# VachaLab/gorder

Measured on AMD Instinct MI355X. Metric: trajectory frames/sec, higher is better.
Workload: dtype f32

## Files before the change

gorder_amd/csrc/kernels_bonds.h:

```cpp
#pragma once

namespace {

__device__ __forceinline__ int grid_index(float x, float lo, float bin, uint32_t n, bool core) {
    const float k = __builtin_roundf(core ? gm_div_core(x - lo, bin) : (x - lo) / bin);
    if (!(k >= 0.0f) || !(k < (float)n)) return -1;
    return (int)k;
}
__device__ __forceinline__ int grid_index_fast(float x, float lo, float inv_bin, uint32_t n) {
    const float k = __builtin_floorf(__builtin_fmaf(x - lo, inv_bin, 0.5f));
    if (!(k >= 0.0f) || !(k < (float)n)) return -1;
    return (int)k;
}
constexpr uint32_t kRecFrames = 4;
struct TiledMapOut {
    uint32_t plane;
    float x0, y0, binx, biny;
    uint32_t nx, ny;
    int bin_core;
    unsigned long long *words;
    unsigned long long *ticks;
};
__device__ __forceinline__ unsigned long long tick_sample_word(int tick, bool lower) {
    return ((unsigned long long)(lower ? 1u : 0u) << 32) | (unsigned long long)(uint32_t)tick;
}
__device__ __forceinline__ unsigned long long map_sample_word(const TiledMapOut &mo, float px, float py, float pz, int tick, bool lower) {
    float x, y;
    if (mo.plane == 0) { x = px; y = py; }
    else if (mo.plane == 1) { x = px; y = pz; }
    else { x = pz; y = py; }
    const int ix = grid_index(x, mo.x0, mo.binx, mo.nx, mo.bin_core != 0), iy = grid_index(y, mo.y0, mo.biny, mo.ny, mo.bin_core != 0);
    if (ix < 0 || iy < 0) return kMapNoSample;
    const uint32_t nt = mo.nx * mo.ny, t = (uint32_t)ix * mo.ny + (uint32_t)iy;
    return ((unsigned long long)((lower ? nt : 0u) + t) << 32) | (unsigned long long)(uint32_t)tick;
}

constexpr uint32_t kNoNan = 0xffffffffu;
struct SampleAcc {
    long long s_tot = 0, s_up = 0;
    uint32_t n_tot = 0, n_up = 0;
};

template <bool ACOS_COS>
__device__ __forceinline__ bool bond_sample(const FrameArgs &a, uint32_t f, float p1x, float p1y, float p1z,
                                            float p2x, float p2y, float p2z, uint32_t mol, SampleAcc &acc,
                                            int &bad, const TiledMapOut *mo = nullptr, unsigned long long *word = nullptr,
                                            unsigned long long *tick_word = nullptr) {
    float vx = p2x - p1x, vy = p2y - p1y, vz = p2z - p1z;
    if (a.pbc) {
        const float *b = a.box9 + 9 * (size_t)f;
        const float bx = b[0], by = b[4], bz = b[8];
        bool slow = false;
        const float rx = gm_min_image_step(vx, bx, slow);
        const float ry = gm_min_image_step(vy, by, slow);
        const float rz = gm_min_image_step(vz, bz, slow);
        if (__builtin_expect(slow, 0)) {
            vx = gm_min_image_loop(vx, bx, bad);
            vy = gm_min_image_loop(vy, by, bad);
            vz = gm_min_image_loop(vz, bz, bad);
        } else {
            vx = rx; vy = ry; vz = rz;
        }
    }
    const float sch = gm_calc_sch<ACOS_COS>(vx, vy, vz, a.nx, a.ny, a.nz, a.n2, a.n2sq);
    const long long tick = gm_tick(sch);
    acc.s_tot += tick;
    acc.n_tot += 1;
    bool lower = false;
    if (a.leaflets) {
        const uint8_t fl = a.aflags[(size_t)a.arow[f] * a.n_mol_total + mol];
        lower = fl != 0;
        if (fl == 0) {
            acc.s_up += tick;
            acc.n_up += 1;
        }
    }
    if (mo) {
        *word = mo->nx == 0u ? tick_sample_word((int)tick, lower)
                             : map_sample_word(*mo, p1x + vx / 2.0f, p1y + vy / 2.0f, p1z + vz / 2.0f, (int)tick, lower);
        if (tick_word) *tick_word = tick_sample_word((int)tick, lower);
    }
    return sch != sch;
}

#ifndef GORDER_COMPUTE_NF
#define GORDER_COMPUTE_NF 8
#endif
typedef float v4f __attribute__((ext_vector_type(4)));

template <int G, int NPF, bool ACOS_COS, bool PBC, bool LEAF, int AXIS = -1>
struct TiledStage {
    static constexpr uint32_t TPF = kBlock / G;

    template <bool TAIL>
    static __device__ __forceinline__ void load(const FrameArgs &a, const Tile &t, uint32_t f0, uint32_t f_end,
                                                uint32_t sk, uint32_t si, v4f (&pre)[NPF]) {
        const uint32_t f = f0 + sk;
        if (TAIL && f >= f_end) return;
        const size_t base = ((size_t)f * a.n_atoms + t.atom0) * 3u;
        const uint32_t n4 = ((uint32_t)(base & 3u) + 3u * t.n_window + 3u) >> 2;
        const v4f *src = reinterpret_cast<const v4f *>(a.xyz + (base & ~(size_t)3));
#pragma unroll
        for (int j = 0; j < NPF; j++) {
            const uint32_t i = si + (uint32_t)j * TPF;
            pre[j] = __builtin_nontemporal_load(src + (i < n4 ? i : n4 - 1u));
        }
    }
    template <bool TAIL, bool FINITE = false>
    static __device__ __forceinline__ bool store(const FrameArgs &a, const Tile &t, uint32_t f0, uint32_t f_end,
                                                 uint32_t sk, uint32_t si, const v4f (&pre)[NPF], float *lds,
                                                 uint32_t lw) {
        const uint32_t f = f0 + sk;
        if (TAIL && f >= f_end) return true;
        const size_t base = ((size_t)f * a.n_atoms + t.atom0) * 3u;
        const uint32_t n4 = ((uint32_t)(base & 3u) + 3u * t.n_window + 3u) >> 2;
        const v4f *src = reinterpret_cast<const v4f *>(a.xyz + (base & ~(size_t)3));
        v4f *dst = reinterpret_cast<v4f *>(lds + (size_t)sk * lw);
        typedef float v2f __attribute__((ext_vector_type(2)));
        v2f poison = {0.0f, 0.0f};
        const v2f zero2 = {0.0f, 0.0f};
#pragma unroll
        for (int j = 0; j < NPF; j++) {
            const uint32_t i = si + (uint32_t)j * TPF;
            if (i < n4) dst[i] = pre[j];
            if (FINITE) {
                poison = __builtin_elementwise_fma(pre[j].xy, zero2, poison);
                poison = __builtin_elementwise_fma(pre[j].zw, zero2, poison);
            }
        }
        for (uint32_t i = si + (uint32_t)NPF * TPF; i < n4; i += TPF) {
            const v4f v = __builtin_nontemporal_load(src + i);
            dst[i] = v;
            if (FINITE) {
                poison = __builtin_elementwise_fma(v.xy, zero2, poison);
                poison = __builtin_elementwise_fma(v.zw, zero2, poison);
            }
        }
        return poison.x + poison.y == 0.0f;
    }
    template <int NF, int OUT = 0>
    static __device__ __forceinline__ void compute_core(const FrameArgs &a, const Tile &t, const Item &it,
                                                        uint32_t f0, const float (&P)[NF][6], SampleAcc &acc,
                                                        int &bad, uint32_t &nan_which, uint32_t &nan_frame,
                                                        const TiledMapOut *mo = nullptr, uint32_t k0 = 0) {
        constexpr bool MAPS = OUT != 0;
        int tick[NF];
        uint8_t fl[NF];
        float bx[NF], by[NF], bz[NF];
        uint32_t rare = 0;
        auto stage_word = [&](int k, float vx, float vy, float vz) {
            mo->words[k0 + (uint32_t)k] = OUT == 2
                ? tick_sample_word(tick[k], LEAF && fl[k] != 0)
                : map_sample_word(*mo, P[k][0] + vx / 2.0f, P[k][1] + vy / 2.0f, P[k][2] + vz / 2.0f, tick[k], LEAF && fl[k] != 0);
            if (OUT == 3) mo->ticks[k0 + (uint32_t)k] = tick_sample_word(tick[k], LEAF && fl[k] != 0);
        };
#pragma unroll
        for (int k = 0; k < NF; k++) {
            if (PBC) {
                const float *b = a.box9 + 9 * (size_t)(f0 + k);
                bx[k] = b[0]; by[k] = b[4]; bz[k] = b[8];
            }
            if (LEAF) fl[k] = a.aflags[(size_t)a.arow[f0 + k] * a.n_mol_total + it.mol];
        }
#pragma unroll
        for (int k = 0; k < NF; k++) {
            float vx = P[k][3] - P[k][0], vy = P[k][4] - P[k][1], vz = P[k][5] - P[k][2];
            bool slow = false;
            if (PBC && AXIS >= 0 && !ACOS_COS && !MAPS) {
                const float ax = __builtin_fabsf(vx), ay = __builtin_fabsf(vy), az = __builtin_fabsf(vz);
                const float tx = bx[k] - ax, ty = by[k] - ay, tz = bz[k] - az;
                vx = ax > bx[k] / 2.0f ? tx : ax;
                vy = ay > by[k] / 2.0f ? ty : ay;
                vz = az > bz[k] / 2.0f ? tz : az;
                slow = __builtin_fminf(__builtin_fminf(tx, ty), tz) < 0.0f;
            } else if (PBC) {
                vx = gm_min_image_step(vx, bx[k], slow);
                vy = gm_min_image_step(vy, by[k], slow);
                vz = gm_min_image_step(vz, bz[k], slow);
            }
            if (AXIS >= 0 && !ACOS_COS) {
                const float sch = gm_sch_axis<AXIS>(vx, vy, vz, slow);
                rare |= (slow ? 1u : 0u) << k;
                tick[k] = gm_tick_finite(sch);
            } else if (AXIS >= 0) {
                const float sch = gm_sch_axis_acos<AXIS>(vx, vy, vz, slow);
                rare |= (slow ? 1u : 0u) << k;
                tick[k] = gm_tick_finite(sch);
            } else {
                bool nonfinite = false;
                const float sch = gm_calc_sch<ACOS_COS, AXIS>(vx, vy, vz, a.nx, a.ny, a.nz, a.n2, a.n2sq, &nonfinite);
                rare |= ((slow || nonfinite || sch != sch) ? 1u : 0u) << k;
                tick[k] = gm_tick(sch);
            }
            if (MAPS) stage_word(k, vx, vy, vz);
        }
        if (__builtin_expect(rare != 0, 0)) {
#pragma unroll
            for (int k = 0; k < NF; k++) {
                if (!((rare >> k) & 1u)) continue;
                float vx = P[k][3] - P[k][0], vy = P[k][4] - P[k][1], vz = P[k][5] - P[k][2];
                if (PBC) {
                    vx = gm_min_image_loop(vx, bx[k], bad);
                    vy = gm_min_image_loop(vy, by[k], bad);
                    vz = gm_min_image_loop(vz, bz[k], bad);
                }
                const float sch = gm_calc_sch<ACOS_COS>(vx, vy, vz, a.nx, a.ny, a.nz, a.n2, a.n2sq);
                tick[k] = gm_tick(sch);
                if (MAPS) stage_word(k, vx, vy, vz);
                if (sch != sch && nan_frame == kNoNan) {
                    if (P[k][0] != P[k][0]) { nan_which = 0; nan_frame = f0 + k; }
                    else if (P[k][3] != P[k][3]) { nan_which = 1; nan_frame = f0 + k; }
                }
            }
        }
        int st = 0, su = 0;
        uint32_t nu = 0;
#pragma unroll
        for (int k = 0; k < NF; k++) {
            st += tick[k];
            if (LEAF) {
                su += fl[k] == 0 ? tick[k] : 0;
                nu += fl[k] == 0 ? 1u : 0u;
            }
        }
        acc.s_tot += st;
        acc.n_tot += NF;
        acc.s_up += su;
        acc.n_up += nu;
    }
    template <int OUT = 0>
    static __device__ __forceinline__ void compute(const FrameArgs &a, const Tile &t, const Item &it, uint32_t f0,
                                                   const float *lds, uint32_t lw, SampleAcc &acc, int &bad,
                                                   uint32_t &nan_which, uint32_t &nan_frame, const TiledMapOut *mo = nullptr) {
        constexpr int NF = (OUT == 1 || OUT == 3 || (OUT == 2 && LEAF)) ? 2 : (GORDER_COMPUTE_NF < G ? GORDER_COMPUTE_NF : G);
#pragma unroll
        for (int h = 0; h < G; h += NF) {
            float P[NF][6];
#pragma unroll
            for (int k = 0; k < NF; k++) {
                const uint32_t sh = (uint32_t)((((size_t)(f0 + h + k) * a.n_atoms + t.atom0) * 3u) & 3u);
                const float *w = lds + (size_t)(h + k) * lw + sh;
                P[k][0] = w[3u * it.li]; P[k][1] = w[3u * it.li + 1]; P[k][2] = w[3u * it.li + 2];
                P[k][3] = w[3u * it.lj]; P[k][4] = w[3u * it.lj + 1]; P[k][5] = w[3u * it.lj + 2];
            }
            compute_core<NF, OUT>(a, t, it, f0 + h, P, acc, bad, nan_which, nan_frame, mo, (uint32_t)h);
        }
    }
    template <int OUT = 0>
    static __device__ __forceinline__ void compute_tail(const FrameArgs &a, const Tile &t, const Item &it,
                                                        uint32_t f0, uint32_t f_end, const float *lds, uint32_t lw,
                                                        SampleAcc &acc, int &bad, uint32_t &nan_which,
                                                        uint32_t &nan_frame, const TiledMapOut *mo = nullptr) {
        if (OUT != 0) {
#pragma unroll
            for (int k = 0; k < G; k++) {
                const uint32_t f = f0 + (uint32_t)k;
                if (f >= f_end) continue;
                const uint32_t sh = (uint32_t)((((size_t)f * a.n_atoms + t.atom0) * 3u) & 3u);
                const float *w = lds + (size_t)k * lw + sh;
                const float p1x = w[3u * it.li], p1y = w[3u * it.li + 1], p1z = w[3u * it.li + 2];
                const float p2x = w[3u * it.lj], p2y = w[3u * it.lj + 1], p2z = w[3u * it.lj + 2];
                if (bond_sample<ACOS_COS>(a, f, p1x, p1y, p1z, p2x, p2y, p2z, it.mol, acc, bad, mo, mo->words + k, OUT == 3 ? mo->ticks + k : nullptr) &&
                    nan_frame == kNoNan) {
                    if (p1x != p1x) { nan_which = 0; nan_frame = f; }
                    else if (p2x != p2x) { nan_which = 1; nan_frame = f; }
                }
            }
            return;
        }
#pragma unroll 1
        for (uint32_t f = f0; f < f_end; f++) {
            const uint32_t sh = (uint32_t)((((size_t)f * a.n_atoms + t.atom0) * 3u) & 3u);
            const float *w = lds + (size_t)(f - f0) * lw + sh;
            const float p1x = w[3u * it.li], p1y = w[3u * it.li + 1], p1z = w[3u * it.li + 2];
            const float p2x = w[3u * it.lj], p2y = w[3u * it.lj + 1], p2z = w[3u * it.lj + 2];
            if (bond_sample<ACOS_COS>(a, f, p1x, p1y, p1z, p2x, p2y, p2z, it.mol, acc, bad) && nan_frame == kNoNan) {
                if (p1x != p1x) { nan_which = 0; nan_frame = f; }
                else if (p2x != p2x) { nan_which = 1; nan_frame = f; }
            }
        }
    }
};

#ifndef GORDER_TILED_MIN_WAVES
#define GORDER_TILED_MIN_WAVES 4
#endif
__device__ __forceinline__ float mom_min(float x, float y) { float r; __asm__("v_min_f32_e32 %0, %1, %2" : "=v"(r) : "v"(x), "v"(y)); return r; }
__device__ __forceinline__ float mom_max(float x, float y) { float r; __asm__("v_max_f32_e32 %0, %1, %2" : "=v"(r) : "v"(x), "v"(y)); return r; }
#define GORDER_MOM_MINMAX_DPP(CTRL_TEXT)                                                                    \
    __asm__("s_nop 1\n\tv_min_f32_dpp %0, %0, %0 " CTRL_TEXT "\n\tv_max_f32_dpp %1, %1, %1 " CTRL_TEXT : "+v"(mn), "+v"(mx))
__device__ __forceinline__ void tiled_moments(const FrameArgs &a, const Tile &t, uint2 own, uint32_t tile_id, uint32_t n_tiles,
                                              uint32_t f, const float *slot, bool finite, uint2 my_head) {
    const uint32_t lane = threadIdx.x & 63u;
    const uint32_t sh = (uint32_t)((((size_t)f * a.n_atoms + t.atom0) * 3u) & 3u);
    const float *w = slot + sh + a.mom_dim + 3u * (own.x - t.atom0);
    const uint32_t n_own = own.y - own.x;
    float s = 0.0f, q = 0.0f, mn = 3.0e38f, mx = -3.0e38f;
    for (uint32_t i0 = 0; i0 < n_own; i0 += 512u) {
        float z[8];
#pragma unroll
        for (uint32_t u = 0; u < 8u; u++) z[u] = w[3u * min(i0 + 64u * u + lane, n_own - 1u)];
#pragma unroll
        for (uint32_t u = 0; u < 8u; u++) {
            if (i0 + 64u * u >= n_own) break;
            float d = z[u];
            if (i0 + 64u * u + 64u > n_own) d = i0 + 64u * u + lane < n_own ? d : 0.0f;
            s += d;
            q = __builtin_fmaf(d, d, q);
            mn = mom_min(mn, z[u]);
            mx = mom_max(mx, z[u]);
        }
    }
#define GORDER_MOM_STEP(CTRL, MASK, CTRL_TEXT)                                                  \
    s += dpp_or_zero<CTRL, MASK>(s); q += dpp_or_zero<CTRL, MASK>(q);                               \
    GORDER_MOM_MINMAX_DPP(CTRL_TEXT);
    GORDER_MOM_STEP(0x111, 0xf, "row_shr:1 row_mask:0xf bank_mask:0xf")
    GORDER_MOM_STEP(0x112, 0xf, "row_shr:2 row_mask:0xf bank_mask:0xf")
    GORDER_MOM_STEP(0x114, 0xf, "row_shr:4 row_mask:0xf bank_mask:0xf")
    GORDER_MOM_STEP(0x118, 0xf, "row_shr:8 row_mask:0xf bank_mask:0xf")
    GORDER_MOM_STEP(0x142, 0xa, "row_bcast:15 row_mask:0xa bank_mask:0xf")
    GORDER_MOM_STEP(0x143, 0xc, "row_bcast:31 row_mask:0xc bank_mask:0xf")
#undef GORDER_MOM_STEP
    const bool all_finite = __all(finite);
    if (lane == 63u) a.mom[(size_t)f * n_tiles + tile_id] = make_float4(all_finite ? s : __builtin_nanf(""), q, mn, mx);
    if (my_head.y != 0xffffffffu) a.head_z[(size_t)f * a.n_mol_total + my_head.y] = slot[sh + a.mom_dim + 3u * my_head.x];
}
template <int G, int NPF, bool ACOS_COS, bool PBC, bool LEAF, int AXIS, bool MOM = false>
__global__ __launch_bounds__(kBlock, GORDER_TILED_MIN_WAVES) void k_bonds_tiled(FrameArgs a_in, const float *__restrict__ xyz,
                                                      const float *__restrict__ box9,
                                                      const uint8_t *__restrict__ aflags,
                                                      const uint32_t *__restrict__ arow,
                                                      const Tile *__restrict__ tiles,
                                                      const Item *__restrict__ items,
                                                      const uint32_t *__restrict__ tile_slots,
                                                      uint32_t n_tiles, uint32_t lw) {
    extern __shared__ __attribute__((aligned(16))) float lds[];
    using S = TiledStage<G, NPF, ACOS_COS, PBC, LEAF, AXIS>;
    FrameArgs a = a_in;
    a.xyz = xyz; a.box9 = box9; a.aflags = aflags; a.arow = arow;
    const uint32_t tile_id = blockIdx.x % n_tiles;
    const uint32_t chunk = blockIdx.x / n_tiles;
    const Tile t = tiles[tile_id];
    const uint32_t tid = threadIdx.x;
    const uint32_t sk = tid / S::TPF, si = tid % S::TPF;
    const bool active = tid < t.n_items;
    Item it{0, 0, 0, 0, 0};
    if (active) it = items[t.item0 + tid];

    const uint32_t f_begin = chunk * a.frames_per_chunk;
    const uint32_t f_end = min(a.n_frames, f_begin + a.frames_per_chunk);
    const uint32_t f_full = f_begin + ((f_end - f_begin) / G) * G;

    SampleAcc acc;
    int bad = 0;
    uint32_t nan_which = 0, nan_frame = kNoNan;
    v4f pre[NPF];
    uint2 own = make_uint2(0u, 0u), my_head = make_uint2(0u, 0xffffffffu);
    if (MOM) {
        own = a.own[tile_id];
        const uint32_t hq = a.own_head_begin[tile_id] + (tid & 63u);
        if (hq < a.own_head_begin[tile_id + 1u]) my_head = a.own_heads[hq];
    }

    if (f_begin < f_full) S::template load<false>(a, t, f_begin, f_end, sk, si, pre);
    for (uint32_t f0 = f_begin; f0 < f_full; f0 += G) {
        const bool finite = S::template store<false, MOM>(a, t, f0, f_end, sk, si, pre, lds, lw);
        __syncthreads();
        if (f0 + G < f_full) S::template load<false>(a, t, f0 + G, f_end, sk, si, pre);
        if (MOM) {
            static_assert(!MOM || (uint32_t)G * 64u == kBlock, "a wave per frame slot");
            tiled_moments(a, t, own, tile_id, n_tiles, f0 + sk, lds + (size_t)sk * lw, finite, my_head);
        }
        if (active) S::compute(a, t, it, f0, lds, lw, acc, bad, nan_which, nan_frame);
        __syncthreads();
    }
    if (f_full < f_end) {
        S::template load<true>(a, t, f_full, f_end, sk, si, pre);
        const bool finite = S::template store<true, MOM>(a, t, f_full, f_end, sk, si, pre, lds, lw);
        __syncthreads();
        if (MOM && f_full + sk < f_end) tiled_moments(a, t, own, tile_id, n_tiles, f_full + sk, lds + (size_t)sk * lw, finite, my_head);
        if (active) S::compute_tail(a, t, it, f_full, f_end, lds, lw, acc, bad, nan_which, nan_frame);
        __syncthreads();
    }

    if (nan_frame != kNoNan)
        raise_error(a.err, GORDER_ERR_UNDEFINED_POSITION, nan_frame, kStageTypes, tile_slots[t.slot0 + it.lslot], 1, it.mol, nan_which);
    if (bad) raise_box_range(a.err, f_begin);

    unsigned long long *l_s = reinterpret_cast<unsigned long long *>(lds);
    uint32_t *l_n = reinterpret_cast<uint32_t *>(l_s + 2 * kBlock);
    l_s[tid] = 0; l_s[kBlock + tid] = 0; l_n[tid] = 0; l_n[kBlock + tid] = 0;
    __syncthreads();
    if (active && acc.n_tot) {
        atomicAdd(&l_s[it.lslot], (unsigned long long)acc.s_tot);
        atomicAdd(&l_n[it.lslot], acc.n_tot);
        if (acc.n_up) {
            atomicAdd(&l_s[kBlock + it.lslot], (unsigned long long)acc.s_up);
            atomicAdd(&l_n[kBlock + it.lslot], acc.n_up);
        }
    }
    __syncthreads();
#ifdef GORDER_DEBUG_NOEPILOGUE
    if (a.n_frames == 0xffffffffu)
#endif
    if (tid < t.n_slots && l_n[tid]) {
        unsigned long long *acc = a.rep + (size_t)(blockIdx.x % a.n_rep) * 4u * a.n_acc;
        const uint32_t slot = tile_slots[t.slot0 + tid];
        atomicAdd(&acc[slot], l_s[tid]);
        atomicAdd(&acc[2u * a.n_acc + slot], (unsigned long long)l_n[tid]);
        if (l_n[kBlock + tid]) {
            atomicAdd(&acc[a.n_acc + slot], l_s[kBlock + tid]);
            atomicAdd(&acc[3u * a.n_acc + slot], (unsigned long long)l_n[kBlock + tid]);
        }
    }
}

template <int G, bool ACOS_COS, bool PBC, bool LEAF>
__global__ __launch_bounds__(kBlock) void k_bonds_gather(FrameArgs a_in, const float *__restrict__ xyz,
                                                       const float *__restrict__ box9,
                                                       const uint8_t *__restrict__ aflags,
                                                       const uint32_t *__restrict__ arow,
                                                       const Tile *__restrict__ tiles,
                                                       const Item *__restrict__ items,
                                                       const uint32_t *__restrict__ tile_slots, uint32_t n_tiles) {
    __shared__ unsigned long long l_s[2 * kBlock];
    __shared__ uint32_t l_n[2 * kBlock];
    using S = TiledStage<G, 1, ACOS_COS, PBC, LEAF>;
    FrameArgs a = a_in;
    a.xyz = xyz; a.box9 = box9; a.aflags = aflags; a.arow = arow;
    const uint32_t tile_id = blockIdx.x % n_tiles;
    const uint32_t chunk = blockIdx.x / n_tiles;
    const Tile t = tiles[tile_id];
    const uint32_t tid = threadIdx.x;
    const bool active = tid < t.n_items;
    Item it{0, 0, 0, 0, 0};
    if (active) it = items[t.item0 + tid];
    const uint32_t f_begin = chunk * a.frames_per_chunk;
    const uint32_t f_end = min(a.n_frames, f_begin + a.frames_per_chunk);
    const uint32_t f_full = f_begin + ((f_end - f_begin) / G) * G;
    const size_t fstride = (size_t)a.n_atoms * 3u;
    const float *pi = xyz + ((size_t)t.atom0 + it.li) * 3u;
    const float *pj = xyz + ((size_t)t.atom0 + it.lj) * 3u;

    SampleAcc acc;
    int bad = 0;
    uint32_t nan_which = 0, nan_frame = kNoNan;
    float cur[G][6], nxt[G][6];
    auto fetch = [&](float (&P)[G][6], uint32_t f0) {
#pragma unroll
        for (int k = 0; k < G; k++) {
            const float *q1 = pi + (size_t)(f0 + k) * fstride, *q2 = pj + (size_t)(f0 + k) * fstride;
            P[k][0] = q1[0]; P[k][1] = q1[1]; P[k][2] = q1[2];
            P[k][3] = q2[0]; P[k][4] = q2[1]; P[k][5] = q2[2];
        }
    };
    if (active) {
        if (f_begin < f_full) fetch(cur, f_begin);
        for (uint32_t f0 = f_begin; f0 < f_full; f0 += G) {
            const bool more = f0 + G < f_full;
            if (more) fetch(nxt, f0 + G);
            S::template compute_core<G>(a, t, it, f0, cur, acc, bad, nan_which, nan_frame);
            if (more) {
#pragma unroll
                for (int k = 0; k < G; k++)
#pragma unroll
                    for (int c = 0; c < 6; c++) cur[k][c] = nxt[k][c];
            }
        }
        for (uint32_t f = f_full; f < f_end; f++) {
            const float *q1 = pi + (size_t)f * fstride, *q2 = pj + (size_t)f * fstride;
            const float p1x = q1[0], p1y = q1[1], p1z = q1[2], p2x = q2[0], p2y = q2[1], p2z = q2[2];
            if (bond_sample<ACOS_COS>(a, f, p1x, p1y, p1z, p2x, p2y, p2z, it.mol, acc, bad) && nan_frame == kNoNan) {
                if (p1x != p1x) { nan_which = 0; nan_frame = f; }
                else if (p2x != p2x) { nan_which = 1; nan_frame = f; }
            }
        }
    }
    if (nan_frame != kNoNan)
        raise_error(a.err, GORDER_ERR_UNDEFINED_POSITION, nan_frame, kStageTypes, tile_slots[t.slot0 + it.lslot], 1, it.mol, nan_which);
    if (bad) raise_box_range(a.err, f_begin);

    l_s[tid] = 0; l_s[kBlock + tid] = 0; l_n[tid] = 0; l_n[kBlock + tid] = 0;
    __syncthreads();
    if (active && acc.n_tot) {
        atomicAdd(&l_s[it.lslot], (unsigned long long)acc.s_tot);
        atomicAdd(&l_n[it.lslot], acc.n_tot);
        if (acc.n_up) {
            atomicAdd(&l_s[kBlock + it.lslot], (unsigned long long)acc.s_up);
            atomicAdd(&l_n[kBlock + it.lslot], acc.n_up);
        }
    }
    __syncthreads();
#ifdef GORDER_DEBUG_NOEPILOGUE
    if (a.n_frames == 0xffffffffu)
#endif
    if (tid < t.n_slots && l_n[tid]) {
        unsigned long long *acc = a.rep + (size_t)(blockIdx.x % a.n_rep) * 4u * a.n_acc;
        const uint32_t slot = tile_slots[t.slot0 + tid];
        atomicAdd(&acc[slot], l_s[tid]);
        atomicAdd(&acc[2u * a.n_acc + slot], (unsigned long long)l_n[tid]);
        if (l_n[kBlock + tid]) {
            atomicAdd(&acc[a.n_acc + slot], l_s[kBlock + tid]);
            atomicAdd(&acc[3u * a.n_acc + slot], (unsigned long long)l_n[kBlock + tid]);
        }
    }
}

template <bool ACOS_COS>
__global__ __launch_bounds__(256) void k_bonds_direct(FrameArgs a, const DirectItem *__restrict__ items,
                                                       uint32_t n_items, uint32_t blocks_per_chunk) {
    const uint32_t chunk = blockIdx.x / blocks_per_chunk;
    const uint32_t q = (blockIdx.x % blocks_per_chunk) * blockDim.x + threadIdx.x;
    if (q >= n_items) return;
    const DirectItem it = items[q];
    const uint32_t f_begin = chunk * a.frames_per_chunk;
    const uint32_t f_end = min(a.n_frames, f_begin + a.frames_per_chunk);
    SampleAcc acc;
    int bad = 0;
    for (uint32_t f = f_begin; f < f_end; f++) {
        const float *p1 = a.xyz + ((size_t)f * a.n_atoms + it.i) * 3u;
        const float *p2 = a.xyz + ((size_t)f * a.n_atoms + it.j) * 3u;
        const float p1x = p1[0], p1y = p1[1], p1z = p1[2];
        const float p2x = p2[0], p2y = p2[1], p2z = p2[2];
        if (__builtin_expect(bond_sample<ACOS_COS>(a, f, p1x, p1y, p1z, p2x, p2y, p2z, it.mol, acc, bad), 0)) {
            if (p1x != p1x) raise_error(a.err, GORDER_ERR_UNDEFINED_POSITION, f, kStageTypes, it.slot, 1, it.mol, 0);
            else if (p2x != p2x) raise_error(a.err, GORDER_ERR_UNDEFINED_POSITION, f, kStageTypes, it.slot, 1, it.mol, 1);
        }
    }
    if (bad) raise_box_range(a.err, f_begin);
    if (acc.n_tot) {
        atomicAdd(&a.acc[it.slot], (unsigned long long)acc.s_tot);
        atomicAdd(&a.acc[2u * a.n_acc + it.slot], (unsigned long long)acc.n_tot);
        if (acc.n_up) {
            atomicAdd(&a.acc[a.n_acc + it.slot], (unsigned long long)acc.s_up);
            atomicAdd(&a.acc[3u * a.n_acc + it.slot], (unsigned long long)acc.n_up);
        }
    }
}

}
```

gorder_amd/csrc/wave_ops.h:

```cpp
#pragma once

namespace {

template <int CTRL, int ROW_MASK = 0xf>
__device__ __forceinline__ int dpp_or_zero(int v) { return __builtin_amdgcn_update_dpp(0, v, CTRL, ROW_MASK, 0xf, true); }
template <int CTRL, int ROW_MASK = 0xf>
__device__ __forceinline__ uint32_t dpp_or_zero(uint32_t v) { return (uint32_t)dpp_or_zero<CTRL, ROW_MASK>((int)v); }
template <int CTRL, int ROW_MASK = 0xf>
__device__ __forceinline__ float dpp_or_zero(float v) { return __int_as_float(dpp_or_zero<CTRL, ROW_MASK>(__float_as_int(v))); }
template <int CTRL, int ROW_MASK = 0xf>
__device__ __forceinline__ double dpp_or_zero(double v) {
    const int lo = dpp_or_zero<CTRL, ROW_MASK>(__double2loint(v)), hi = dpp_or_zero<CTRL, ROW_MASK>(__double2hiint(v));
    return __hiloint2double(hi, lo);
}
template <int CTRL, int ROW_MASK = 0xf>
__device__ __forceinline__ unsigned long long dpp_or_zero(unsigned long long v) {
    const uint32_t lo = dpp_or_zero<CTRL, ROW_MASK>((uint32_t)v), hi = dpp_or_zero<CTRL, ROW_MASK>((uint32_t)(v >> 32));
    return ((unsigned long long)hi << 32) | lo;
}
template <int CTRL, int ROW_MASK = 0xf>
__device__ __forceinline__ float dpp_or_self(float v) {
    return __int_as_float(__builtin_amdgcn_update_dpp(__float_as_int(v), __float_as_int(v), CTRL, ROW_MASK, 0xf, false));
}
__device__ __forceinline__ int lane_value(int v, int l) { return __builtin_amdgcn_readlane(v, l); }
__device__ __forceinline__ uint32_t lane_value(uint32_t v, int l) { return (uint32_t)__builtin_amdgcn_readlane((int)v, l); }
__device__ __forceinline__ float lane_value(float v, int l) { return __int_as_float(__builtin_amdgcn_readlane(__float_as_int(v), l)); }
__device__ __forceinline__ double lane_value(double v, int l) {
    return __hiloint2double(__builtin_amdgcn_readlane(__double2hiint(v), l), __builtin_amdgcn_readlane(__double2loint(v), l));
}
__device__ __forceinline__ unsigned long long lane_value(unsigned long long v, int l) {
    return ((unsigned long long)lane_value((uint32_t)(v >> 32), l) << 32) | lane_value((uint32_t)v, l);
}

template <class T>
__device__ __forceinline__ T row_sum(T v) {
    v = v + dpp_or_zero<0x111>(v); v = v + dpp_or_zero<0x112>(v); v = v + dpp_or_zero<0x114>(v); v = v + dpp_or_zero<0x118>(v);
    return v;
}
template <int CTRL, class... T>
__device__ __forceinline__ void row_step(T &...v) { ((v = v + dpp_or_zero<CTRL>(v)), ...); }
template <class... T>
__device__ __forceinline__ void row_sums(T &...v) { row_step<0x111>(v...); row_step<0x112>(v...); row_step<0x114>(v...); row_step<0x118>(v...); }
template <class T>
__device__ __forceinline__ T rows_to_wave(T v) {
    v = v + dpp_or_zero<0x142, 0xa>(v); v = v + dpp_or_zero<0x143, 0xc>(v);
    return v;
}
template <class T>
__device__ __forceinline__ T wave_sum_rows(T v) { return lane_value(rows_to_wave(row_sum(v)), 63); }
__device__ __forceinline__ float wave_min_rows(float v) {
    v = fminf(v, dpp_or_self<0x111>(v)); v = fminf(v, dpp_or_self<0x112>(v));
    v = fminf(v, dpp_or_self<0x114>(v)); v = fminf(v, dpp_or_self<0x118>(v));
    v = fminf(v, dpp_or_self<0x142, 0xa>(v)); v = fminf(v, dpp_or_self<0x143, 0xc>(v));
    return lane_value(v, 63);
}
__device__ __forceinline__ float wave_max_rows(float v) {
    v = fmaxf(v, dpp_or_self<0x111>(v)); v = fmaxf(v, dpp_or_self<0x112>(v));
    v = fmaxf(v, dpp_or_self<0x114>(v)); v = fmaxf(v, dpp_or_self<0x118>(v));
    v = fmaxf(v, dpp_or_self<0x142, 0xa>(v)); v = fmaxf(v, dpp_or_self<0x143, 0xc>(v));
    return lane_value(v, 63);
}
__device__ __forceinline__ uint32_t wave_scan_rows(uint32_t v, uint32_t lane) {
    v = row_sum(v);
    const uint32_t t0 = lane_value(v, 15), t1 = lane_value(v, 31), t2 = lane_value(v, 47);
    const uint32_t r = lane >> 4;
    return v + (r > 0u ? t0 : 0u) + (r > 1u ? t1 : 0u) + (r > 2u ? t2 : 0u);
}
__device__ __forceinline__ unsigned long long wave_scan_rows(unsigned long long v, uint32_t lane) {
    v = row_sum(v);
    const unsigned long long t0 = lane_value(v, 15), t1 = lane_value(v, 31), t2 = lane_value(v, 47);
    const uint32_t r = lane >> 4;
    return v + (r > 0u ? t0 : 0ull) + (r > 1u ? t1 : 0ull) + (r > 2u ? t2 : 0ull);
}
__device__ __forceinline__ double wave_scan_rows(double v, uint32_t lane) {
    v = row_sum(v);
    const double t0 = lane_value(v, 15), t1 = lane_value(v, 31), t2 = lane_value(v, 47);
    const uint32_t r = lane >> 4;
    return v + (r > 0u ? t0 : 0.0) + (r > 1u ? t1 : 0.0) + (r > 2u ? t2 : 0.0);
}

__device__ __forceinline__ double wave_sum_bfly(double v) {
    for (int off = 32; off > 0; off >>= 1) v += __shfl_xor(v, off, 64);
    return v;
}
__device__ __forceinline__ uint32_t wave_max_bfly(uint32_t v) {
    for (int off = 32; off > 0; off >>= 1) v = max(v, (uint32_t)__shfl_xor((int)v, off, 64));
    return v;
}
__device__ __forceinline__ void wave_minmax_bfly(float &lo, float &hi) {
    for (int off = 32; off > 0; off >>= 1) {
        lo = fminf(lo, __shfl_xor(lo, off, 64));
        hi = fmaxf(hi, __shfl_xor(hi, off, 64));
    }
}
__device__ __forceinline__ void wave_minmax_or_bfly(float &lo, float &hi, uint32_t &flags) {
    for (int off = 32; off >= 1; off >>= 1) {
        lo = fminf(lo, __shfl_xor(lo, off, 64));
        hi = fmaxf(hi, __shfl_xor(hi, off, 64));
        flags |= (uint32_t)__shfl_xor((int)flags, off, 64);
    }
}
__device__ __forceinline__ void wave_sum2_minmax_bfly(double &s, double &q, float &lo, float &hi) {
    for (int off = 32; off >= 1; off >>= 1) {
        s += __shfl_xor(s, off, 64); q += __shfl_xor(q, off, 64);
        lo = fminf(lo, __shfl_xor(lo, off, 64)); hi = fmaxf(hi, __shfl_xor(hi, off, 64));
    }
}
__device__ __forceinline__ uint32_t wave_scan_shfl(uint32_t v, uint32_t lane) {
    for (uint32_t off = 1; off < 64u; off <<= 1) {
        const uint32_t t = __shfl_up(v, off, 64);
        if (lane >= off) v += t;
    }
    return v;
}

template <int N>
__device__ __forceinline__ void block_sum_n(double (&v)[N], double *scratch) {
    const uint32_t wave = threadIdx.x >> 6, n_waves = (blockDim.x + 63u) >> 6;
#pragma unroll
    for (int q = 0; q < N; q++) {
        v[q] = wave_sum_bfly(v[q]);
        if ((threadIdx.x & 63u) == 0) scratch[16 * q + wave] = v[q];
    }
    __syncthreads();
#pragma unroll
    for (int q = 0; q < N; q++) {
        double r = 0.0;
        for (uint32_t w = 0; w < n_waves; w++) r += scratch[16 * q + w];
        v[q] = r;
    }
    __syncthreads();
}
__device__ __forceinline__ double block_sum(double v, double *scratch ) {
    double a[1] = {v};
    block_sum_n<1>(a, scratch);
    return a[0];
}
__device__ __forceinline__ void block_minmax(float &lo, float &hi, float *scratch ) {
    wave_minmax_bfly(lo, hi);
    const uint32_t wave = threadIdx.x >> 6, n_waves = (blockDim.x + 63u) >> 6;
    if ((threadIdx.x & 63u) == 0) { scratch[wave] = lo; scratch[16 + wave] = hi; }
    __syncthreads();
    for (uint32_t w = 0; w < n_waves; w++) { lo = fminf(lo, scratch[w]); hi = fmaxf(hi, scratch[16 + w]); }
    __syncthreads();
}

__device__ __forceinline__ uint32_t local_float_key(float v) {
    const uint32_t b = __float_as_uint(v);
    return (b & 0x80000000u) ? ~b : (b | 0x80000000u);
}
__device__ __forceinline__ float local_key_float(uint32_t k) {
    return __uint_as_float((k & 0x80000000u) ? (k & 0x7fffffffu) : ~k);
}
__device__ __forceinline__ void block_finfo_record(float zlo, float zhi, uint32_t &flags, uint32_t record_mask, float *l_lo,
                                                   float *l_hi, uint32_t *l_flags, uint4 *out) {
    wave_minmax_or_bfly(zlo, zhi, flags);
    const uint32_t tid = threadIdx.x;
    if ((tid & 63u) == 0u) { l_lo[tid >> 6] = zlo; l_hi[tid >> 6] = zhi; l_flags[tid >> 6] = flags; }
    __syncthreads();
    if (tid == 0u) {
        for (uint32_t w = 1; w < 16u; w++) { zlo = fminf(zlo, l_lo[w]); zhi = fmaxf(zhi, l_hi[w]); flags |= l_flags[w]; }
        *out = zlo <= zhi ? make_uint4(local_float_key(zlo), local_float_key(zhi), flags & record_mask, 2u)
                          : make_uint4(0xffffffffu, 0u, flags & record_mask, 2u);
    }
}

}
```

Baseline: 21.01 million.

## Fold wave moment reduction into paired halves via permlane32 swap

Replaces four independent 64-lane DPP reductions (sum, sum of squares, min, max) with a folded scheme. Min is turned into a max of negated values, lanes are remapped so that a permlane32 swap packs two quantities into one register per half-wave, and a single 32-lane DPP chain then reduces sum/q and max/-min together. This roughly halves the DPP reduction instruction count, at the cost of a lane remapping for the loads and extra readlanes to pull the results out.

Measured after the change: 20.50 million. -2.4%, worse.

```diff
diff --git a/gorder_amd/csrc/kernels_bonds.h b/gorder_amd/csrc/kernels_bonds.h
--- a/gorder_amd/csrc/kernels_bonds.h
+++ b/gorder_amd/csrc/kernels_bonds.h
@@ -285,44 +285,35 @@
 #ifndef GORDER_TILED_MIN_WAVES
 #define GORDER_TILED_MIN_WAVES 4
 #endif
-__device__ __forceinline__ float mom_min(float x, float y) { float r; __asm__("v_min_f32_e32 %0, %1, %2" : "=v"(r) : "v"(x), "v"(y)); return r; }
 __device__ __forceinline__ float mom_max(float x, float y) { float r; __asm__("v_max_f32_e32 %0, %1, %2" : "=v"(r) : "v"(x), "v"(y)); return r; }
-#define GORDER_MOM_MINMAX_DPP(CTRL_TEXT)                                                                    \
-    __asm__("s_nop 1\n\tv_min_f32_dpp %0, %0, %0 " CTRL_TEXT "\n\tv_max_f32_dpp %1, %1, %1 " CTRL_TEXT : "+v"(mn), "+v"(mx))
+__device__ __forceinline__ float mom_max_neg(float x, float y) { float r; __asm__("v_max_f32_e64 %0, %1, -%2" : "=v"(r) : "v"(x), "v"(y)); return r; }
 __device__ __forceinline__ void tiled_moments(const FrameArgs &a, const Tile &t, uint2 own, uint32_t tile_id, uint32_t n_tiles,
                                               uint32_t f, const float *slot, bool finite, uint2 my_head) {
-    const uint32_t lane = threadIdx.x & 63u;
+    const uint32_t lane = threadIdx.x & 63u, mine = folded_slot(lane);
     const uint32_t sh = (uint32_t)((((size_t)f * a.n_atoms + t.atom0) * 3u) & 3u);
     const float *w = slot + sh + a.mom_dim + 3u * (own.x - t.atom0);
     const uint32_t n_own = own.y - own.x;
-    float s = 0.0f, q = 0.0f, mn = 3.0e38f, mx = -3.0e38f;
+    float s = 0.0f, q = 0.0f, nmn = -3.0e38f, mx = -3.0e38f;
     for (uint32_t i0 = 0; i0 < n_own; i0 += 512u) {
         float z[8];
 #pragma unroll
-        for (uint32_t u = 0; u < 8u; u++) z[u] = w[3u * min(i0 + 64u * u + lane, n_own - 1u)];
+        for (uint32_t u = 0; u < 8u; u++) z[u] = w[3u * min(i0 + 64u * u + mine, n_own - 1u)];
 #pragma unroll
         for (uint32_t u = 0; u < 8u; u++) {
             if (i0 + 64u * u >= n_own) break;
             float d = z[u];
-            if (i0 + 64u * u + 64u > n_own) d = i0 + 64u * u + lane < n_own ? d : 0.0f;
+            if (i0 + 64u * u + 64u > n_own) d = i0 + 64u * u + mine < n_own ? d : 0.0f;
             s += d;
             q = __builtin_fmaf(d, d, q);
-            mn = mom_min(mn, z[u]);
+            nmn = mom_max_neg(nmn, z[u]);
             mx = mom_max(mx, z[u]);
         }
     }
-#define GORDER_MOM_STEP(CTRL, MASK, CTRL_TEXT)                                                  \
-    s += dpp_or_zero<CTRL, MASK>(s); q += dpp_or_zero<CTRL, MASK>(q);                               \
-    GORDER_MOM_MINMAX_DPP(CTRL_TEXT);
-    GORDER_MOM_STEP(0x111, 0xf, "row_shr:1 row_mask:0xf bank_mask:0xf")
-    GORDER_MOM_STEP(0x112, 0xf, "row_shr:2 row_mask:0xf bank_mask:0xf")
-    GORDER_MOM_STEP(0x114, 0xf, "row_shr:4 row_mask:0xf bank_mask:0xf")
-    GORDER_MOM_STEP(0x118, 0xf, "row_shr:8 row_mask:0xf bank_mask:0xf")
-    GORDER_MOM_STEP(0x142, 0xa, "row_bcast:15 row_mask:0xa bank_mask:0xf")
-    GORDER_MOM_STEP(0x143, 0xc, "row_bcast:31 row_mask:0xc bank_mask:0xf")
-#undef GORDER_MOM_STEP
+    float sum, top;
+    wave_sum2_max2_folded(s, q, nmn, mx, sum, top);
+    const float s_all = lane_value(sum, 31), nmn_all = lane_value(top, 31);
     const bool all_finite = __all(finite);
-    if (lane == 63u) a.mom[(size_t)f * n_tiles + tile_id] = make_float4(all_finite ? s : __builtin_nanf(""), q, mn, mx);
+    if (lane == 63u) a.mom[(size_t)f * n_tiles + tile_id] = make_float4(all_finite ? s_all : __builtin_nanf(""), sum, -nmn_all, top);
     if (my_head.y != 0xffffffffu) a.head_z[(size_t)f * a.n_mol_total + my_head.y] = slot[sh + a.mom_dim + 3u * my_head.x];
 }
 template <int G, int NPF, bool ACOS_COS, bool PBC, bool LEAF, int AXIS, bool MOM = false>
diff --git a/gorder_amd/csrc/wave_ops.h b/gorder_amd/csrc/wave_ops.h
--- a/gorder_amd/csrc/wave_ops.h
+++ b/gorder_amd/csrc/wave_ops.h
@@ -59,6 +59,26 @@
     v = fmaxf(v, dpp_or_self<0x114>(v)); v = fmaxf(v, dpp_or_self<0x118>(v));
     v = fmaxf(v, dpp_or_self<0x142, 0xa>(v)); v = fmaxf(v, dpp_or_self<0x143, 0xc>(v));
     return lane_value(v, 63);
+}
+__device__ __forceinline__ uint32_t folded_slot(uint32_t lane) {
+    const uint32_t j = lane & 31u;
+    return 2u * j + ((lane >> 5) ^ (j >> 4));
+}
+__device__ __forceinline__ void wave_sum2_max2_folded(float s, float q, float e, float f, float &sum, float &top) {
+    const auto sq = __builtin_amdgcn_permlane32_swap(__float_as_uint(s), __float_as_uint(q), false, false);
+    const auto ef = __builtin_amdgcn_permlane32_swap(__float_as_uint(e), __float_as_uint(f), false, false);
+    sum = __uint_as_float(sq[0]) + __uint_as_float(sq[1]);
+    top = __uint_as_float(ef[0]);
+    const float other = __uint_as_float(ef[1]);
+#define GORDER_FOLDED_STEP(CTRL_TEXT) "s_nop 0\n\tv_add_f32_dpp %0, %0, %0 " CTRL_TEXT "\n\tv_max_f32_dpp %1, %1, %1 " CTRL_TEXT "\n\t"
+    __asm__("v_max_f32_e32 %1, %1, %2\n\t"
+            GORDER_FOLDED_STEP("row_shr:1 row_mask:0xf bank_mask:0xf")
+            GORDER_FOLDED_STEP("row_shr:2 row_mask:0xf bank_mask:0xf")
+            GORDER_FOLDED_STEP("row_shr:4 row_mask:0xf bank_mask:0xf")
+            GORDER_FOLDED_STEP("row_shr:8 row_mask:0xf bank_mask:0xf")
+            GORDER_FOLDED_STEP("row_bcast:15 row_mask:0xa bank_mask:0xf")
+            : "+v"(sum), "+v"(top) : "v"(other));
+#undef GORDER_FOLDED_STEP
 }
 __device__ __forceinline__ uint32_t wave_scan_rows(uint32_t v, uint32_t lane) {
     v = row_sum(v);
```
